# thelaycon/lazzaro

Hardware: AMD Instinct MI355X
Metric: search_memories QPS + recall@10 on 10M x d=768 index; consolidate turns/sec (higher is better)
Workload: dtype bf16 encoder; int8 scan -> bf16 re-score -> fp32 re-rank; 1 GPU; global_batch=1024, seq_len=32, parallelism=tenant-dp1

## Files before the change

csrc/kernels/search256.hip:

```cpp
#include "lzk_g256.h"
#include "lzk_i8score.h"

#include <cstdlib>
#include <cfloat>
#include <map>
#include <mutex>

LZK_DEBUG_STATE(search256)

namespace {

using namespace g256;

constexpr int kStampTiles = 32;
__device__ unsigned long long* g_stamps = nullptr;

template <bool HAS_BIAS, bool HAS_LABEL>
__global__ __launch_bounds__(NT, 1) void flat_cand_kernel(
    const u16* __restrict__ X, long ldx, int nrows, const u16* __restrict__ Qm, long ldq, int nq, int D,
    const float* __restrict__ bias, const int* __restrict__ row_label, const int* __restrict__ q_label,
    float alpha, const float* __restrict__ thr, int n_qt, int cap, int* __restrict__ cnt,
    float* __restrict__ cs, int* __restrict__ ci) {
  extern __shared__ __attribute__((aligned(16))) u16 smem[];
  const int logical = xcd_remap(blockIdx.x, gridDim.x);
// ... 554 lines not shown
    int mr = 0x7fffffff;
#pragma unroll
    for (int i = 0; i < 8; ++i) {
      const int rb = r0 + wr * 128 + i * 16 + 4 * (lane >> 4);
#pragma unroll
      for (int e = 0; e < 4; ++e) {
        const float v = acc[i][j][e];
        if (rb + e < nrows && v > m) { m = v; mr = rb + e; }
      }
    }
#pragma unroll
    for (int off = 16; off <= 32; off <<= 1) {
      const float om = __shfl_xor(m, off);
      const int orr = __shfl_xor(mr, off);
      if (om > m || (om == m && orr < mr)) { m = om; mr = orr; }
    }
    const int q = q0 + wc * 64 + j * 16 + (lane & 15);
    if ((lane >> 4) == 0 && q < nq && mr < nrows) atomicMax(best + q, top1_pack(m, mr));
  }
}

__global__ __launch_bounds__(NT, 1) void flat_top1_grouped_kernel(const u16* __restrict__ C, long ldc,
                                                                  const u16* __restrict__ Xq, long ldx,
                                                                  const int* __restrict__ qidx,
                                                                  const int4* __restrict__ blocks, int D,
                                                                  unsigned long long* __restrict__ best) {
  extern __shared__ __attribute__((aligned(16))) u16 smem[];
  const int4 bd = blocks[xcd_remap(blockIdx.x, gridDim.x)];
  const int c0 = bd.x, nc = bd.y, p0 = bd.z, np = bd.w;
  Stager st;
  st.setup(C + (long)c0 * ldc, ldc, 0, nc, Xq, ldx, 0, 1);
  {
    const int wave = __builtin_amdgcn_readfirstlane(threadIdx.x >> 6);
    const int lane = threadIdx.x & 63;
#pragma unroll
    for (int i = 0; i < 2; ++i) {
      const int row = 8 * (wave * 2 + i) + (lane >> 3);
      const int kc = (lane & 7) ^ ((row >> 1) & 7);
      LZK_DCHECK(qidx[p0 + min(row, np - 1)] >= 0);
      st.src[2][i] = Xq + (long)qidx[p0 + min(row, np - 1)] * ldx + kc * 8;
      st.src[3][i] = Xq + (long)qidx[p0 + min(128 + row, np - 1)] * ldx + kc * 8;
    }
  }
  f32x4 acc[8][4];
  mainloop(smem, st, D / BK, acc);

  const int lane = threadIdx.x & 63;
  const int wave = __builtin_amdgcn_readfirstlane(threadIdx.x >> 6);
  const int wr = wave >> 2, wc = wave & 3;
#pragma unroll
  for (int j = 0; j < 4; ++j) {
    float m = LZK_NEG_INF;
    int mr = 0x7fffffff;
#pragma unroll
    for (int i = 0; i < 8; ++i) {
      const int rb = wr * 128 + i * 16 + 4 * (lane >> 4);
#pragma unroll
      for (int e = 0; e < 4; ++e) {
        const float v = acc[i][j][e];
        if (rb + e < nc && v > m) { m = v; mr = rb + e; }
      }
    }
#pragma unroll
    for (int off = 16; off <= 32; off <<= 1) {
      const float om = __shfl_xor(m, off);
      const int orr = __shfl_xor(mr, off);
      if (om > m || (om == m && orr < mr)) { m = om; mr = orr; }
    }
    const int q = wc * 64 + j * 16 + (lane & 15);
    if ((lane >> 4) == 0 && q < np && mr < nc) atomicMax(best + p0 + q, top1_pack(m, c0 + mr));
  }
}

__global__ __launch_bounds__(256) void top1_decode_kernel(const unsigned long long* __restrict__ best, int nq,
                                                          float* __restrict__ score, int* __restrict__ row) {
  const int q = blockIdx.x * 256 + threadIdx.x;
  if (q >= nq) return;
  const unsigned long long b = best[q];
  if (b == 0ull) { score[q] = LZK_NEG_INF; row[q] = -1; return; }
  const unsigned key = (unsigned)(b >> 32);
  const unsigned u = (key & 0x80000000u) ? (key & 0x7fffffffu) : ~key;
  score[q] = __uint_as_float(u);
  row[q] = (int)(0xFFFFFFFFu - (unsigned)(b & 0xFFFFFFFFull));
}

template <bool F32>
__device__ __forceinline__ void load4(const void* p, long off, float (&v)[4]) {
  if constexpr (F32) {
    const float4 u = *reinterpret_cast<const float4*>(reinterpret_cast<const float*>(p) + off);
    v[0] = u.x; v[1] = u.y; v[2] = u.z; v[3] = u.w;
  } else {
    const uint2 u = *reinterpret_cast<const uint2*>(reinterpret_cast<const u16*>(p) + off);
    v[0] = __uint_as_float(u.x << 16); v[1] = __uint_as_float(u.x & 0xffff0000u);
    v[2] = __uint_as_float(u.y << 16); v[3] = __uint_as_float(u.y & 0xffff0000u);
  }
}

template <bool F32>
__global__ __launch_bounds__(256) void cand_rescore_kernel(const void* __restrict__ X, long ldx,
                                                           const void* __restrict__ Qm, long ldq, int D,
                                                           const float* __restrict__ bias, float alpha,
                                                           const int* __restrict__ cnt, int cap,
                                                           float* __restrict__ cs, const int* __restrict__ ci,
                                                           const float* __restrict__ cut, float floor,
                                                           const float* __restrict__ tau, int k_need,
                                                           int need_val, int* __restrict__ need,
                                                           int* __restrict__ hitc, int* __restrict__ done) {
  __shared__ int s_hits;
  const int q = blockIdx.x;
  const int lane = threadIdx.x & 63, wave = threadIdx.x >> 6;
  const int split = gridDim.y;
  if (threadIdx.x == 0) s_hits = 0;
  __syncthreads();
  const float tq = tau ? tau[q] : LZK_NEG_INF;
  int hits = 0;
  const int n = min(cnt[q] & 0x3fffffff, cap);
  const int chunks = D >> 2;
  constexpr int MAXC = 8;
  float qv[MAXC][4];
#pragma unroll
  for (int t = 0; t < MAXC; ++t) {
    const int c = lane + 64 * t;
    if (c < chunks) load4<F32>(Qm, (long)q * ldq + 4 * c, qv[t]);
  }
  const float cq = cut ? cut[q] : LZK_NEG_INF;
  for (int base = blockIdx.y * 256 + wave * 64; base < n; base += 256 * split) {
    const long li = (long)q * cap + base + lane;
    bool keep = base + lane < n;
    if (keep && cut) {
      keep = cs[li] >= cq;
      if (!keep) cs[li] = LZK_NEG_INF;
    }
    unsigned long long live = __ballot(keep);
    while (live) {
    const int jj = __builtin_ctzll(live);
    live &= live - 1;
    const long idx = (long)q * cap + base + jj;
    const int r = ci[idx];
    LZK_DCHECK(r >= 0);
    float acc = 0.f;
#pragma unroll
    for (int t = 0; t < MAXC; ++t) {
      const int c = lane + 64 * t;
      if (c < chunks) {
        float xv[4];
        load4<F32>(X, (long)r * ldx + 4 * c, xv);
        acc = fmaf(qv[t][0], xv[0], acc);
        acc = fmaf(qv[t][1], xv[1], acc);
        acc = fmaf(qv[t][2], xv[2], acc);
        acc = fmaf(qv[t][3], xv[3], acc);
      }
    }
#pragma unroll
    for (int o = 32; o >= 1; o >>= 1) acc += __shfl_xor(acc, o, 64);
    const float sc = alpha * acc + (bias ? bias[r] : 0.f);
    if (lane == 0) cs[idx] = sc >= floor ? sc : LZK_NEG_INF;
    hits += (sc >= floor && sc >= tq) ? 1 : 0;
    }
  }
  if (need) {
    if (lane == 0 && hits) atomicAdd(&s_hits, hits);
    __syncthreads();
    if (threadIdx.x == 0) {
      int tot = s_hits;
      bool last = true;
      if (split > 1) {
// ... 515 lines not shown
    if (hipMalloc(&s.p, (size_t)cap * sizeof(int)) != hipSuccess) {
      s.cap = 0;
      return nullptr;
    }
    s.cap = cap;
  }
  if (hipMemsetAsync(s.p, 0, (size_t)2 * nq * sizeof(int), st) != hipSuccess) return nullptr;
  return s.p;
}

template <bool F32>
int launch_rescore(const void* X, long ldx, const void* Q, long ldq, int nq, int D, const float* bias, float alpha,
                   const int* cnt, int cap, float* cs, const int* ci, const float* cut, float floor, const float* tau,
                   int k_need, int need_val, int* need, hipStream_t st) {
  int split = rescore_split(nq);
  int* ctr = nullptr;
  if (split > 1 && need) {
    ctr = rescore_counters(nq, st);
    if (!ctr) split = 1;
  }
  if (split > 1)
    hipLaunchKernelGGL(cand_rescore4_kernel<F32>, dim3((unsigned)nq, (unsigned)split), dim3(256), 0, st, X, ldx, Q,
                       ldq, D, bias, alpha, cnt, cap, cs, ci, cut, floor, tau, k_need, need_val, need, ctr,
                       ctr ? ctr + nq : nullptr);
  else
    hipLaunchKernelGGL(cand_rescore_kernel<F32>, dim3((unsigned)nq, 1u), dim3(256), 0, st, X, ldx, Q, ldq, D, bias,
                       alpha, cnt, cap, cs, ci, cut, floor, tau, k_need, need_val, need, ctr, ctr ? ctr + nq : nullptr);
  return (int)hipGetLastError();
}
}

LZK_EXPORT int lzk_cand_rescore(const void* X16, long ldx, const void* Q16, long ldq, int nq, int D, const float* bias,
                                float alpha, const int* cnt, int cap, float* cs, const int* ci, const float* cut,
                                float floor, const float* tau, int k_need, int need_val, int* need, void* stream) {
  if (D % 4 != 0 || D > 2048 || nq <= 0) return (int)hipErrorInvalidValue;
  return launch_rescore<false>(X16, ldx, Q16, ldq, nq, D, bias, alpha, cnt, cap, cs, ci, cut, floor, tau, k_need,
                               need_val, need, (hipStream_t)stream);
}

LZK_EXPORT int lzk_cand_rescore32(const float* X32, long ldx, const float* Q32, long ldq, int nq, int D,
                                  const float* bias, float alpha, const int* cnt, int cap, float* cs, const int* ci,
                                  const float* cut, float floor, const float* tau, int k_need, int need_val,
                                  int* need, void* stream) {
  if (D % 4 != 0 || D > 2048 || nq <= 0 || ldx % 4 != 0 || ldq % 4 != 0) return (int)hipErrorInvalidValue;
  return launch_rescore<true>(X32, ldx, Q32, ldq, nq, D, bias, alpha, cnt, cap, cs, ci, cut, floor, tau, k_need,
                              need_val, need, (hipStream_t)stream);
}

__global__ __launch_bounds__(256) void thr_prep_kernel(const float* __restrict__ ts, long ldts, int col,
                                                       const float* __restrict__ margin,
                                                       const float* __restrict__ margin_rig, int nq,
                                                       float* __restrict__ thr, float* __restrict__ cert,
                                                       int* __restrict__ cnt) {
#pragma clang fp contract(off)
  const int q = blockIdx.x * 256 + threadIdx.x;
  if (q >= nq) return;
  float t = ts[(long)q * ldts + col];
  const float sl = 1.0f + fabsf(t);
  t = t - 2e-4f * sl;
  if (t != t) t = LZK_NEG_INF;
  else if (t == LZK_NEG_INF) t = -FLT_MAX;
  else if (t == __builtin_inff()) t = FLT_MAX;
  const float th = margin ? t - margin[q] : t;
  thr[q] = th;
  if (cert) {
    float c = margin_rig ? th + margin_rig[q] : th;
    const float cs = 1.0f + fabsf(c);
    c = c + 1e-6f * cs;
    if (c != c) c = LZK_NEG_INF;
    else if (c == __builtin_inff()) c = FLT_MAX;
    cert[q] = c;
  }
  if (cnt) cnt[q] = 0;
}

LZK_EXPORT int lzk_thr_prep(const float* ts, long ldts, int col, const float* margin, const float* margin_rig, int nq,
                            float* thr, float* cert, int* cnt, void* stream) {
  if (nq <= 0 || col < 0 || col >= ldts || !ts || !thr) return (int)hipErrorInvalidValue;
  hipLaunchKernelGGL(thr_prep_kernel, dim3((unsigned)((nq + 255) / 256)), dim3(256), 0, (hipStream_t)stream, ts, ldts,
                     col, margin, margin_rig, nq, thr, cert, cnt);
  return (int)hipGetLastError();
}

LZK_EXPORT int lzk_cand_cut(const void* X, long ldx, long nrows, const void* Q, long ldq, int D, int nq, int f32,
                            const float* bias, float alpha, const long* rows, int ldr, int k, const float* margin,
                            float floor, int has_floor, float* cut, void* stream) {
  if (D % 4 != 0 || D > 2048 || nq <= 0 || k <= 0 || k > ldr || !margin) return (int)hipErrorInvalidValue;
  if (f32 && (ldx % 4 != 0 || ldq % 4 != 0)) return (int)hipErrorInvalidValue;
  const dim3 grid((unsigned)((nq + 3) / 4)), block(256);
  if (nq < 64 && k <= 16) {
    if (f32)
      hipLaunchKernelGGL(cand_cut_block_kernel<true>, dim3((unsigned)nq), dim3(1024), 0, (hipStream_t)stream, X, ldx,
                         nrows, Q, ldq, D, nq, bias, alpha, rows, ldr, k, margin, floor, has_floor, cut);
    else
      hipLaunchKernelGGL(cand_cut_block_kernel<false>, dim3((unsigned)nq), dim3(1024), 0, (hipStream_t)stream, X,
                         ldx, nrows, Q, ldq, D, nq, bias, alpha, rows, ldr, k, margin, floor, has_floor, cut);
    return (int)hipGetLastError();
  }
  if (f32)
    hipLaunchKernelGGL(cand_cut_kernel<true>, grid, block, 0, (hipStream_t)stream, X, ldx, nrows, Q, ldq, D, nq,
                       bias, alpha, rows, ldr, k, margin, floor, has_floor, cut);
  else
    hipLaunchKernelGGL(cand_cut_kernel<false>, grid, block, 0, (hipStream_t)stream, X, ldx, nrows, Q, ldq, D, nq,
                       bias, alpha, rows, ldr, k, margin, floor, has_floor, cut);
  return (int)hipGetLastError();
}

LZK_EXPORT int lzk_flat_cand_i8(const void* X8, long ldx_bytes, int nrows, const void* Q8, long ldq_bytes, int nq,
                                int D_bytes, const float* bias, const float* rscale, const float* qscale, float alpha,
                                const float* thr, int cap, int* cnt, float* cs, int* ci, void* blk_buf, int blk_cap,
                                int* blk_cnt, void* stream) {
  if (D_bytes % 128 != 0 || D_bytes > 1024 || (ldx_bytes | ldq_bytes) % 16 != 0 || nq <= 0 || nrows <= 0 ||
      cap <= 0 || !rscale || !qscale || !(alpha > 0.f))
    return (int)hipErrorInvalidValue;
  if (!blk_buf || blk_cap <= 0 || !blk_cnt) return (int)hipErrorInvalidValue;
  const BlkCands blk{(int4*)blk_buf, blk_cap, blk_cnt, rscale, qscale};
  const int n_rt = (nrows + BM - 1) / BM, n_qt = (nq + BN - 1) / BN;
  const long nblk = (long)n_rt * n_qt;
  if (nblk > 0x7fffffffL) return (int)hipErrorInvalidValue;
  const int ncu = n_cu();
  const int grid = (int)(nblk < ncu ? nblk : ncu);
  hipStream_t st = (hipStream_t)stream;
  const u16* x = (const u16*)X8;
  const u16* q = (const u16*)Q8;
  const int* rs = nullptr;
  const int* qs = nullptr;
#define LZK_GIO(B, O)                                                                                               \
  do {                                                                                                              \
    (void)hipFuncSetAttribute((const void*)flat_cand_persistent_kernel<B, false, false, O, MmaI8>,                  \
                              hipFuncAttributeMaxDynamicSharedMemorySize, CAND_P_LDS);                              \
    hipLaunchKernelGGL((flat_cand_persistent_kernel<B, false, false, O, MmaI8>), dim3(grid), dim3(NT), CAND_P_LDS, \
                       st, x, ldx_bytes / 2, nrows, q, ldq_bytes / 2, nq, D_bytes / 2, bias, rs, qs, alpha, thr,    \
                       n_qt, (int)nblk, cap, cnt, cs, ci, (const float*)nullptr, (int*)nullptr, (float*)nullptr,    \
                       (int*)nullptr, blk);                                                                         \
  } while (0)
#define LZK_GIS(B)                              \
  do {                                          \
    switch (g_i8_opt) {                         \
      case 28: LZK_GIO(B, 28); break;           \
      case 8: LZK_GIO(B, 8); break;             \
      case 24: LZK_GIO(B, 24); break;           \
      case 88: LZK_GIO(B, 88); break;           \
      default: LZK_GIO(B, kI8Opt); break;       \
    }                                           \
  } while (0)
  if (bias) LZK_GIS(true);
  else LZK_GIS(false);
#undef LZK_GIS
#undef LZK_GIO
  return (int)hipGetLastError();
}

LZK_EXPORT int lzk_flat_cand_dual_i8(const void* X8, long ldx_bytes, int nrows, const void* Q8, long ldq_bytes,
                                     int nq, int D_bytes, const float* bias, const float* rscale,
                                     const float* qscale, const int* row_label, const int* q_label, float alpha,
                                     const float* thr, const float* thr2, int cap, int* cnt, float* cs, int* ci,
                                     int* cnt2, float* cs2, int* ci2, void* blk_buf, int blk_cap, int* blk_cnt,
                                     void* stream) {
  if (D_bytes % 128 != 0 || D_bytes > 1024 || (ldx_bytes | ldq_bytes) % 16 != 0 || nq <= 0 || nrows <= 0 ||
      cap <= 0 || !rscale || !qscale || !row_label || !q_label || !(alpha > 0.f))
    return (int)hipErrorInvalidValue;
  if (!blk_buf || blk_cap <= 0 || !blk_cnt) return (int)hipErrorInvalidValue;
  const BlkCands blk{(int4*)blk_buf, blk_cap, blk_cnt, rscale, qscale};
  const int n_rt = (nrows + BM - 1) / BM, n_qt = (nq + BN - 1) / BN;
  const long nblk = (long)n_rt * n_qt;
  if (nblk > 0x7fffffffL) return (int)hipErrorInvalidValue;
// ... 29 lines not shown
```

lazzaro_amd/ops/search.py:

```python
from __future__ import annotations

import math
import os

import numpy as np
import torch

from . import _lib

TARGET_WGS = 512


def _ref_topk(X, Q, k, bias=None, row_label=None, q_label=None, alpha=1.0, idx_offset=0,
              chunk=1 << 16):
    nq = Q.shape[0]
    n = X.shape[0]
    dev = X.device
    best_s = torch.full((nq, 0), float("-inf"), device=dev)
    best_i = torch.zeros((nq, 0), dtype=torch.long, device=dev)
    Qf = Q.float()
    for c0 in range(0, n, chunk):
        c1 = min(n, c0 + chunk)
        s = alpha * (Qf @ X[c0:c1].float().T)
        if bias is not None:
# ... 391 lines not shown
    thr = _sample_threshold(X16, Q16, k, kslot, bias, None, None, alpha, S)
    if margin is not None:
        thr = (thr - margin).contiguous()
    cap = max(2048, 32 * kslot * S)
    cnt, cs, ci = _cand_lists(dev, nq, cap, 0)
    grid = L.lzk_cand_grid_f8(N, nq)
    bbuf, bcap, bcnt = _blk_records(dev, grid, nq, kslot, 4 * S, 1)
    st = _lib.stream_ptr(dev)
    _lib.check(L.lzk_flat_cand_f8(X8.data_ptr(), X8.stride(0), N, Q8.data_ptr(), Q8.stride(0), nq, Dp, _lib.ptr(bias),
                                  float(alpha / scale2), thr.data_ptr(), cap, cnt.data_ptr(), cs.data_ptr(),
                                  ci.data_ptr(), bbuf.data_ptr(), bcap, bcnt.data_ptr(), st), "lzk_flat_cand_f8")
    _lib.check(L.lzk_cand_gather(bbuf.data_ptr(), bcap, bcnt.data_ptr(), grid, cap, nq, cnt.data_ptr(), cs.data_ptr(),
                                 ci.data_ptr(), None, None, None, st), "lzk_cand_gather")
    _lib.check(L.lzk_cand_rescore(X16.data_ptr(), X16.stride(0), Q16.data_ptr(), Q16.stride(0), nq, Dp,
                                  _lib.ptr(bias), float(alpha), cnt.data_ptr(), cap, cs.data_ptr(), ci.data_ptr(), None,
                                  float("-inf"), None, 0, 0, None, st), "lzk_cand_rescore")
    return _select_with_fallback(X16, Q16, k, kslot, bias, None, None, alpha, 0, cnt, cs, ci, cap)


def quantize_i8_rows(x: torch.Tensor, out: torch.Tensor = None, scale_out: torch.Tensor = None):
    xf = x.float()
    amax = xf.abs().amax(1)
    s = torch.where(amax > 0, amax / 127.0, torch.zeros_like(amax))
    den = torch.where(amax > 0, s, torch.ones_like(amax))
    q = torch.round(xf / den[:, None]).clamp_(-127, 127).to(torch.int8)
    if out is not None:
        out[:, : q.shape[1]] = q
        q = out
    if scale_out is not None:
        scale_out.copy_(s)
        s = scale_out
    return q, s


def i8_query(q16: torch.Tensor, d: int, sumsq: torch.Tensor, n_sumsq: int, smax: torch.Tensor, alpha: float,
             z: float, xn: float = 1.0):
    nq, Dp = q16.shape
    dev = q16.device
    q8 = torch.empty((nq, Dp), dtype=torch.int8, device=dev)
    qs = torch.empty(nq, dtype=torch.float32, device=dev)
    margin = torch.empty(nq, dtype=torch.float32, device=dev)
    margin_rig = torch.empty(nq, dtype=torch.float32, device=dev)
    q16 = q16.contiguous()
    _lib.check(_lib.lib().lzk_i8_query(q16.data_ptr(), q16.stride(0), nq, Dp, int(d), sumsq.data_ptr(),
                                       1.0 / max(int(n_sumsq), 1), smax.data_ptr(), abs(float(alpha)), float(z),
                                       float(xn), q8.data_ptr(), q8.stride(0), qs.data_ptr(), margin.data_ptr(),
                                       margin_rig.data_ptr(), _lib.stream_ptr(dev)), "lzk_i8_query")
    return q8, qs, margin, margin_rig


I8_SAMPLE = os.environ.get("LZK_I8_SAMPLE", "1") != "0"
_lib.register("lzk_sample_topk_i8", _lib.I, [_lib.P, _lib.L, _lib.I, _lib.I, _lib.P, _lib.L, _lib.I, _lib.P, _lib.P,
                                             _lib.P, _lib.F, _lib.I, _lib.I, _lib.I, _lib.P, _lib.P, _lib.P])


def sample_topk_i8(X8: torch.Tensor, rscale: torch.Tensor, Q8: torch.Tensor, qscale: torch.Tensor, kslot: int,
                   S: int, *, bias=None, alpha: float = 1.0, n_chunks: int = None):
    L = _lib.lib()
    nq, Dp = Q8.shape
    N = X8.shape[0]
    dev = X8.device
    assert X8.dtype == torch.int8 and Q8.dtype == torch.int8 and Dp % 128 == 0 and Dp <= 1024 and X8.shape[1] == Dp
    assert X8.stride(1) == 1 and Q8.stride(1) == 1 and N > 0 and nq > 0 and S >= 1
    assert rscale.dtype == torch.float32 and rscale.stride(0) == 1 and rscale.shape[0] >= N
    assert bias is None or (bias.dtype == torch.float32 and bias.stride(0) == 1 and bias.shape[0] >= N)
    qs = qscale.contiguous()
    assert qs.dtype == torch.float32 and qs.shape[0] == nq
    ns = -(-N // S)
    if n_chunks:
        rpc = -(-(-(-ns // n_chunks)) // 128) * 128
        nch = -(-ns // rpc)
    else:
        nch = L.lzk_flat_topk_chunks(ns, nq, TARGET_WGS)
    part = nq * nch * kslot
    ws = _ws.get(dev, part * 8)
    ps = ws[: part * 4].view(torch.float32)
    pi = ws[part * 4: part * 8].view(torch.int32)
    _lib.check(L.lzk_sample_topk_i8(X8.data_ptr(), X8.stride(0), N, int(S), Q8.data_ptr(), Q8.stride(0), nq,
                                    rscale.data_ptr(), qs.data_ptr(), _lib.ptr(bias), float(alpha), Dp, kslot, nch,
                                    ps.data_ptr(), pi.data_ptr(), _lib.stream_ptr(dev)), "lzk_sample_topk_i8")
    return _merge_partials(ps, pi, nch, nq, kslot, kslot, 0)


def flat_topk_i8(X8: torch.Tensor, rscale: torch.Tensor, Q8: torch.Tensor, qscale: torch.Tensor,
                 X16: torch.Tensor, Q16: torch.Tensor, k: int, *, bias=None, alpha: float = 1.0, margin=None,
                 margin_rig=None):
    L = _lib.lib()
    nq, Dp = Q16.shape
    N = X16.shape[0]
    kslot = L.lzk_flat_topk_kslot(int(k))
    assert kslot > 0 and X8.dtype == torch.int8 and Q8.dtype == torch.int8 and Dp % 128 == 0 and Dp <= 1024
    assert X8.shape[1] == Dp and X8.stride(1) == 1 and Q8.stride(1) == 1 and X8.shape[0] >= N
    assert rscale.dtype == torch.float32 and qscale.dtype == torch.float32 and rscale.shape[0] >= N
    assert alpha > 0
    dev = X16.device
    if margin_rig is None:
        margin_rig = margin
    narrow = nq < NARROW_MAX_Q and SCAN8_NARROW and Dp % 64 == 0
    S = max(1, min(CAND_STRIDE_NARROW if narrow else CAND_STRIDE, N // max(16 * kslot, 1)))
    J = SPEC_J_NARROW if narrow else SPEC_J
    spec = 0 < J < k and S >= SPEC_MIN_STRIDE
    if I8_SAMPLE:
        ts, _ = sample_topk_i8(X8[:N], rscale, Q8, qscale, kslot, S, bias=bias, alpha=alpha)
    else:
        bs = bias[:N:S].contiguous() if bias is not None else None
        ts, _ = _flat_topk_lane(X16[::S], Q16, kslot, kslot, bs, None, None, alpha, 0, None)
    cap = max(NARROW_CAP if narrow else 2048, 16 * kslot * S)
    cnt, cs, ci = _cand_lists(dev, nq, cap, 0, zero=False)
    thr = torch.empty(nq, dtype=torch.float32, device=dev)
    cert = torch.empty(nq, dtype=torch.float32, device=dev)
    mg = margin.float().contiguous() if margin is not None else None
    mr = margin_rig.float().contiguous() if margin_rig is not None else None
    _lib.check(L.lzk_thr_prep(ts.data_ptr(), ts.stride(0), (J if spec else k) - 1, _lib.ptr(mg), _lib.ptr(mr), nq,
                              thr.data_ptr(), cert.data_ptr(), cnt.data_ptr(), _lib.stream_ptr(dev)), "lzk_thr_prep")
    qs = qscale.contiguous()
    need = torch.empty(nq, dtype=torch.int32, device=dev)
    chk = (cert, k, cap + 1, need)
    if narrow:
        _scan8_narrow(X8[:N], rscale[:N], Q8, qs, bias, alpha, thr, kslot, 2 * S, cap, (cnt, cs, ci))
    else:
        grid = L.lzk_cand_grid_f8(N, nq)
        bbuf, bcap, bcnt = _blk_records(dev, grid, nq, kslot, 2 * S, 1)
        st = _lib.stream_ptr(dev)
        _lib.check(L.lzk_flat_cand_i8(X8.data_ptr(), X8.stride(0), N, Q8.data_ptr(), Q8.stride(0), nq, Dp,
                                      _lib.ptr(bias), rscale.data_ptr(), qs.data_ptr(), float(alpha), thr.data_ptr(),
                                      cap, cnt.data_ptr(), cs.data_ptr(), ci.data_ptr(), bbuf.data_ptr(), bcap,
                                      bcnt.data_ptr(), st), "lzk_flat_cand_i8")
        _lib.check(L.lzk_cand_gather(bbuf.data_ptr(), bcap, bcnt.data_ptr(), grid, cap, nq, cnt.data_ptr(),
                                     cs.data_ptr(), ci.data_ptr(), None, None, None, st), "lzk_cand_gather")
    _rescore_above_cut(X16, Q16, k, kslot, bias, alpha, margin_rig, cnt, cs, ci, cap, chk=chk)
    return _select_with_fallback(X16, Q16, k, kslot, bias, None, None, alpha, 0, cnt, cs, ci, cap, need=need)


_lib.register("lzk_cand_select_wide", _lib.I, [_lib.P, _lib.P, _lib.P, _lib.I, _lib.I, _lib.I, _lib.L, _lib.P, _lib.P,
                                               _lib.P, _lib.P, _lib.P, _lib.P])
_lib.register("lzk_flat_topk_wide_chunks", _lib.I, [_lib.I, _lib.I])
_lib.register("lzk_flat_topk_wide", _lib.I, [_lib.P, _lib.L, _lib.I, _lib.P, _lib.L, _lib.I, _lib.P, _lib.F, _lib.I,
                                             _lib.I, _lib.P, _lib.P, _lib.I, _lib.L, _lib.P, _lib.P, _lib.P])
_lib.register("lzk_flat_topk_wide_masked", _lib.I, [_lib.P, _lib.L, _lib.I, _lib.P, _lib.L, _lib.I, _lib.P, _lib.F,
                                                    _lib.I, _lib.I, _lib.P, _lib.P, _lib.I, _lib.L, _lib.P, _lib.P,
                                                    _lib.P, _lib.P])

WIDE_K_MAX = 64
WIDE_P_FALLBACK = 1e-4
WIDE_J = None
WIDE_CAP_MIN = 2048
WIDE_LIST_FACTOR = 16
_ws_wide = _Workspace()


def wide_spec_j(k: int, S: int, p_max: float = WIDE_P_FALLBACK) -> int:
    k, S = int(k), max(int(S), 1)
    p = 1.0 / S
    for j in range(1, 17):
        tail = sum(math.comb(k, i) * p ** i * (1.0 - p) ** (k - i) for i in range(j, k + 1))
        if tail <= p_max:
            return j
    return 16


def _wide_chunks(N: int, nq: int, n_chunks=None) -> int:
    hint = int(n_chunks) if n_chunks else min(-(-N // 8192), max(8, min(256, 65536 // max(nq, 1))))
    return _lib.lib().lzk_flat_topk_wide_chunks(int(N), max(hint, 1))


def _flat_topk_wide(X16, Q16, k, bias, alpha, idx_offset=0, n_chunks=None, q_active=None, out=None):
    L = _lib.lib()
    nq, D = Q16.shape
    N = X16.shape[0]
    dev = X16.device
    assert X16.dtype == torch.bfloat16 and Q16.dtype == torch.bfloat16 and 1 <= k <= WIDE_K_MAX
    assert X16.shape[1] == D and D % 8 == 0 and D <= 2048 and X16.stride(1) == 1 and Q16.stride(1) == 1
    assert bias is None or (bias.dtype == torch.float32 and bias.is_contiguous() and bias.shape[0] >= N)
    if out is None:
        assert q_active is None
        out = (torch.empty((nq, k), dtype=torch.float32, device=dev), torch.empty((nq, k), dtype=torch.long, device=dev))
    os_, oi = out
    nch = _wide_chunks(N, nq, n_chunks)
    part = nq * nch * WIDE_K_MAX
    ws = _ws_wide.get(dev, part * 8)
    ps = ws[: part * 4].view(torch.float32)
    pi = ws[part * 4: part * 8].view(torch.int32)
    args = (X16.data_ptr(), X16.stride(0), N, Q16.data_ptr(), Q16.stride(0), nq, _lib.ptr(bias), float(alpha), D,
            nch, ps.data_ptr(), pi.data_ptr(), int(k), int(idx_offset), os_.data_ptr(), oi.data_ptr())
    if q_active is None:
        _lib.check(L.lzk_flat_topk_wide(*args, _lib.stream_ptr(dev)), "lzk_flat_topk_wide")
    else:
        assert q_active.dtype == torch.int32 and q_active.shape[0] == nq
        _lib.check(L.lzk_flat_topk_wide_masked(*args, q_active.data_ptr(), _lib.stream_ptr(dev)),
                   "lzk_flat_topk_wide_masked")
    return os_, oi


def flat_topk_wide(X16: torch.Tensor, Q16: torch.Tensor, k: int, *, bias=None, alpha: float = 1.0,
                   idx_offset: int = 0, n_chunks: int = None):
    if Q16.dim() == 1:
        Q16 = Q16[None, :]
    if not X16.is_cuda:
        return _ref_topk(X16, Q16, k, bias, None, None, alpha, idx_offset)
    nq = Q16.shape[0]
    if X16.shape[0] == 0 or nq == 0:
        return (torch.full((nq, k), float("-inf"), device=X16.device),
                torch.full((nq, k), -1, dtype=torch.long, device=X16.device))
    return _flat_topk_wide(X16, Q16, k, bias, alpha, idx_offset, n_chunks)


def cand_select_wide(cnt, cs, ci, cap: int, kout: int, *, idx_offset: int = 0, need=None, q_active=None, out=None):
    nq = cs.shape[0] if cs.dim() == 2 else cs.numel() // cap
    dev = cs.device
    if out is None:
        out = (torch.empty((nq, kout), dtype=torch.float32, device=dev),
               torch.empty((nq, kout), dtype=torch.long, device=dev))
    ovf = torch.empty((nq,), dtype=torch.int32, device=dev)
    _lib.check(_lib.lib().lzk_cand_select_wide(_lib.ptr(cnt), cs.data_ptr(), ci.data_ptr(), int(cap), nq, int(kout),
                                               int(idx_offset), out[0].data_ptr(), out[1].data_ptr(), ovf.data_ptr(),
                                               _lib.ptr(need), _lib.ptr(q_active), _lib.stream_ptr(dev)),
               "lzk_cand_select_wide")
    return out[0], out[1], ovf


def flat_topk_i8_wide(X8: torch.Tensor, rscale: torch.Tensor, Q8: torch.Tensor, qscale: torch.Tensor,
                      X16: torch.Tensor, Q16: torch.Tensor, k: int, *, bias=None, alpha: float = 1.0, margin=None,
                      margin_rig=None):
    k = int(k)
    assert 16 < k <= WIDE_K_MAX, "flat_topk_i8_wide serves 17 <= k <= 64 (flat_topk_i8 below)"
    if not X16.is_cuda:
        return _ref_topk(X16, Q16, k, bias, None, None, alpha, 0)
    L = _lib.lib()
    nq, Dp = Q16.shape
    N = X16.shape[0]
    kslot = 16
    assert X8.dtype == torch.int8 and Q8.dtype == torch.int8 and Dp % 128 == 0 and Dp <= 1024
    assert X8.shape[1] == Dp and X8.stride(1) == 1 and Q8.stride(1) == 1 and X8.shape[0] >= N
    assert rscale.dtype == torch.float32 and qscale.dtype == torch.float32 and rscale.shape[0] >= N
    assert alpha > 0 and not isinstance(X16, LeanRows)
    dev = X16.device
    st = _lib.stream_ptr(dev)
    if margin_rig is None:
        margin_rig = margin
    narrow = nq < NARROW_MAX_Q and SCAN8_NARROW and Dp % 64 == 0
    S = max(1, min(CAND_STRIDE_NARROW if narrow else CAND_STRIDE, N // max(16 * kslot, 1)))
    j = int(WIDE_J) if WIDE_J else wide_spec_j(k, S)
    ts, _ = sample_topk_i8(X8[:N], rscale, Q8, qscale, kslot, S, bias=bias, alpha=alpha)
    cap = max(NARROW_CAP if narrow else WIDE_CAP_MIN, WIDE_LIST_FACTOR * j * S, WIDE_K_MAX)
    cnt, cs, ci = _cand_lists(dev, nq, cap, 0, zero=False)
    thr = torch.empty(nq, dtype=torch.float32, device=dev)
    cert = torch.empty(nq, dtype=torch.float32, device=dev)
    mg = margin.float().contiguous() if margin is not None else None
    mr = margin_rig.float().contiguous() if margin_rig is not None else None
    _lib.check(L.lzk_thr_prep(ts.data_ptr(), ts.stride(0), j - 1, _lib.ptr(mg), _lib.ptr(mr), nq, thr.data_ptr(),
                              cert.data_ptr(), cnt.data_ptr(), st), "lzk_thr_prep")
    qs = qscale.contiguous()
    need = torch.empty(nq, dtype=torch.int32, device=dev)
    if narrow:
        _scan8_narrow(X8[:N], rscale[:N], Q8, qs, bias, alpha, thr, j, 2 * S, cap, (cnt, cs, ci))
    else:
        grid = L.lzk_cand_grid_f8(N, nq)
        bbuf, bcap, bcnt = _blk_records(dev, grid, nq, j, 2 * S, 1)
        _lib.check(L.lzk_flat_cand_i8(X8.data_ptr(), X8.stride(0), N, Q8.data_ptr(), Q8.stride(0), nq, Dp,
                                      _lib.ptr(bias), rscale.data_ptr(), qs.data_ptr(), float(alpha), thr.data_ptr(),
                                      cap, cnt.data_ptr(), cs.data_ptr(), ci.data_ptr(), bbuf.data_ptr(), bcap,
                                      bcnt.data_ptr(), st), "lzk_flat_cand_i8")
        _lib.check(L.lzk_cand_gather(bbuf.data_ptr(), bcap, bcnt.data_ptr(), grid, cap, nq, cnt.data_ptr(),
                                     cs.data_ptr(), ci.data_ptr(), None, None, None, st), "lzk_cand_gather")
    _rescore_above_cut_wide(X16, Q16, k, bias, alpha, mr, cnt, cs, ci, cap, (cert, k, cap + 1, need))
    return _select_with_fallback_wide(X16, Q16, k, bias, alpha, cnt, cs, ci, cap, need=need)


def _rescore_above_cut_wide(X16, Q16, k, bias, alpha, margin, cnt, cs, ci, cap, chk):
    L = _lib.lib()
    nq, Dp = Q16.shape
    dev = Q16.device
    st = _lib.stream_ptr(dev)
    tau, k_need, need_val, need = chk
    cut = None
    if margin is not None:
        _, i8, _ = cand_select_wide(cnt, cs, ci, cap, k)
        cut = torch.empty(nq, dtype=torch.float32, device=dev)
        _lib.check(L.lzk_cand_cut(X16.data_ptr(), X16.stride(0), int(X16.shape[0]), Q16.data_ptr(), Q16.stride(0),
                                  Dp, nq, 0, _lib.ptr(bias), float(alpha), i8.data_ptr(), k, k, margin.data_ptr(),
                                  0.0, 0, cut.data_ptr(), st), "lzk_cand_cut")
    _lib.check(L.lzk_cand_rescore(X16.data_ptr(), X16.stride(0), Q16.data_ptr(), Q16.stride(0), nq, Dp,
                                  _lib.ptr(bias), float(alpha), cnt.data_ptr(), cap, cs.data_ptr(), ci.data_ptr(),
                                  _lib.ptr(cut), float("-inf"), tau.data_ptr(), int(k_need), int(need_val),
                                  need.data_ptr(), st), "lzk_cand_rescore")


def _select_with_fallback_wide(X16, Q16, k, bias, alpha, cnt, cs, ci, cap, need=None, ovf_sink=None):
    os_, oi, ovf = cand_select_wide(cnt, cs, ci, cap, k, need=need)
    if ovf_sink is not None:
        ovf_sink.append((ovf, cnt))
    return _flat_topk_wide(X16, Q16, k, bias, alpha, 0, None, q_active=ovf, out=(os_, oi))


def _cert_tau(thr: torch.Tensor, margin_rig: torch.Tensor, floor: float = None,
              floor_tol: float = 0.0) -> torch.Tensor:
    t = thr + margin_rig if margin_rig is not None else thr
    fl_ok = (t <= float(floor) + float(floor_tol)) if floor is not None else None
    t = t + 1e-6 * (1.0 + t.abs())
    if fl_ok is not None:
        t = torch.where(fl_ok, torch.full_like(t, float("-inf")), t)
    return torch.nan_to_num(t, nan=float("-inf"), neginf=float("-inf")).contiguous()


SPEC_J = 5
SPEC_J_NARROW = 3
NARROW_CAP = 16384
SPEC_MIN_STRIDE = 32
SPEC_STATS = [] if os.environ.get("LZK_SPEC_STATS") == "1" else None


def _rescore_above_cut(X16, Q16, k, kslot, bias, alpha, margin, cnt, cs, ci, cap, floor=None, chk=None):
    tau_p, k_need, need_val, need_p = (None, 0, 0, None) if chk is None else (
        chk[0].data_ptr(), int(chk[1]), int(chk[2]), chk[3].data_ptr())
    L = _lib.lib()
    nq, Dp = Q16.shape
    dev = Q16.device
    st = _lib.stream_ptr(dev)
    cut = None
    if margin is not None:
        s8 = torch.empty((nq, kslot), dtype=torch.float32, device=dev)
        i8 = torch.empty((nq, kslot), dtype=torch.long, device=dev)
        ovf = torch.empty((nq,), dtype=torch.int32, device=dev)
        _lib.check(L.lzk_cand_select(cnt.data_ptr(), cs.data_ptr(), ci.data_ptr(), cap, nq, kslot, kslot, 0,
                                     s8.data_ptr(), i8.data_ptr(), ovf.data_ptr(), None, st), "lzk_cand_select")
        cut = torch.empty(nq, dtype=torch.float32, device=dev)
# ... 341 lines not shown
```

Baseline: 85750 queries/s.

## Replace sampled top-k threshold with per-group max then select

Adds a sampled int8 GEMM kernel that writes only a per-128-row-group maximum score per query, instead of full per-chunk top-k partials. A small select kernel then picks the top kslot group maxima to form the threshold. The goal is to cut the cost of the sampling stage (partial top-k maintenance and the merge). The resulting threshold is a lower bound that differs from the true k-th sampled score, which may let more candidates through the later stages. It is enabled by default when there are enough groups, and the epilogue scales and bias are staged into LDS asynchronously.

```diff
diff --git a/csrc/kernels/search256.hip b/csrc/kernels/search256.hip
--- a/csrc/kernels/search256.hip
+++ b/csrc/kernels/search256.hip
@@ -660,6 +660,152 @@
   const unsigned u = (key & 0x80000000u) ? (key & 0x7fffffffu) : ~key;
   score[q] = __uint_as_float(u);
   row[q] = (int)(0xFFFFFFFFu - (unsigned)(b & 0xFFFFFFFFull));
+}
+
+constexpr int GMAX_ARRAYS = 3;
+constexpr int GMAX_LDS = LDS_BYTES + 2 * GMAX_ARRAYS * 256 * 4;
+
+template <bool HAS_BIAS, bool STAGED>
+__global__ __launch_bounds__(NT, 1) void sample_gmax_i8_kernel(
+    const u16* __restrict__ X, long lds_row, int ns, long S, const u16* __restrict__ Qm, long ldq, int nq, int D,
+    const float* __restrict__ rscale, const float* __restrict__ bias, const float* __restrict__ qscale, float alpha,
+    int n_qt, int n_tiles, float* __restrict__ gmax, long ldg) {
+  typedef int i32x4 __attribute__((ext_vector_type(4)));
+  extern __shared__ __attribute__((aligned(16))) u16 smem[];
+  float* epi = reinterpret_cast<float*>(smem + EPI_OFF);
+  const int lane = threadIdx.x & 63;
+  const int wave = __builtin_amdgcn_readfirstlane(threadIdx.x >> 6);
+  const int wr = wave >> 2, wc = wave & 3;
+  const int KS = D / BK;
+
+  TileWalk walk;
+  walk.init(n_tiles);
+  int tile = walk.next;
+  if (!walk.valid(tile)) return;
+
+  auto stage_epi = [&](int tl, int par) {
+    if constexpr (STAGED) {
+      const int r0 = (tl / n_qt) * BM, q0 = (tl % n_qt) * BN;
+#pragma unroll
+      for (int g = wave; g < 4 * GMAX_ARRAYS; g += 8) {
+        const int a = g >> 2, c = g & 3;
+        if (a == 1 && !HAS_BIAS) continue;
+        const long r = (long)min(r0 + c * 64 + lane, ns - 1) * S;
+        const float* src;
+        if (a == 0) src = rscale + r;
+        else if (a == 1) src = bias + r;
+        else src = qscale + min(q0 + c * 64 + lane, nq - 1);
+        __builtin_amdgcn_global_load_lds((gbl_void_t*)src,
+                                         (lds_void_t*)(epi + par * (GMAX_ARRAYS * 256) + a * 256 + c * 64), 4, 0, 0);
+      }
+    }
+  };
+
+  Stager st;
+  st.setup(X, lds_row, (tile / n_qt) * BM, ns, Qm, ldq, (tile % n_qt) * BN, nq);
+  auto ex0 = [&]() { stage_epi(tile, 0); };
+  prologue<decltype(ex0), 8>(smem, st, KS, ex0);
+  int par = 0;
+  f32x4 acc[8][4];
+  while (true) {
+    const int cur = tile, cpar = par;
+    tile += walk.step;
+    const bool more = walk.valid(tile);
+    body2<MmaI8>(smem, st, KS, acc, true);
+    if (more) {
+      st.setup(X, lds_row, (tile / n_qt) * BM, ns, Qm, ldq, (tile % n_qt) * BN, nq);
+      auto exn = [&]() { stage_epi(tile, cpar ^ 1); };
+      prologue<decltype(exn), 8>(smem, st, KS, exn);
+    }
+    const int r0 = (cur / n_qt) * BM, q0 = (cur % n_qt) * BN;
+    const float* e_rs = epi + cpar * (GMAX_ARRAYS * 256);
+    const float* e_bias = e_rs + 256;
+    const float* e_qs = e_rs + 512;
+    const bool full = r0 + BM <= ns;
+    float al[4], m[4];
+#pragma unroll
+    for (int j = 0; j < 4; ++j) {
+      const int qlo = wc * 64 + j * 16 + (lane & 15);
+      al[j] = alpha * (STAGED ? e_qs[qlo] : qscale[min(q0 + qlo, nq - 1)]);
+      m[j] = LZK_NEG_INF;
+    }
+#pragma unroll
+    for (int i = 0; i < 8; ++i) {
+      const int rl = wr * 128 + i * 16 + 4 * (lane >> 4);
+      f32x4 rs, bv = {0.f, 0.f, 0.f, 0.f};
+      if constexpr (STAGED) {
+        rs = *reinterpret_cast<const f32x4*>(e_rs + rl);
+        if (HAS_BIAS) bv = *reinterpret_cast<const f32x4*>(e_bias + rl);
+      } else {
+#pragma unroll
+        for (int e = 0; e < 4; ++e) {
+          const long r = (long)min(r0 + rl + e, ns - 1) * S;
+          rs[e] = rscale[r];
+          if (HAS_BIAS) bv[e] = bias[r];
+        }
+      }
+#pragma unroll
+      for (int j = 0; j < 4; ++j) {
+        const i32x4 v = __builtin_bit_cast(i32x4, acc[i][j]);
+#pragma unroll
+        for (int e = 0; e < 4; ++e) {
+          float sc = i8_score(al[j], i8_prod(v[e], rs[e]), bv[e]);
+          if (!(full || r0 + rl + e < ns)) sc = LZK_NEG_INF;
+          m[j] = fmaxf(m[j], sc);
+        }
+      }
+    }
+    float* out = gmax + (long)(2 * (r0 / BM) + wr) * ldg;
+#pragma unroll
+    for (int j = 0; j < 4; ++j) {
+      float mm = fmaxf(m[j], __shfl_xor(m[j], 16, 64));
+      mm = fmaxf(mm, __shfl_xor(mm, 32, 64));
+      const int q = q0 + wc * 64 + j * 16 + (lane & 15);
+      if ((lane >> 4) == 0 && q < nq) out[q] = mm;
+    }
+    if (!more) break;
+    par = cpar ^ 1;
+  }
+}
+
+template <int K>
+__global__ __launch_bounds__(256) void gmax_select_kernel(const float* __restrict__ gmax, long ldg, int G, int nq,
+                                                          float* __restrict__ ts) {
+  const int lane = threadIdx.x & 63;
+  const int q = blockIdx.x * 4 + (threadIdx.x >> 6);
+  if (q >= nq) return;
+  TopK<K> top;
+  top.init();
+  constexpr int U = 8;
+  for (int g0 = 0; g0 < G; g0 += 64 * U) {
+    float v[U];
+#pragma unroll
+    for (int u = 0; u < U; ++u) {
+      const int g = g0 + u * 64 + lane;
+      v[u] = g < G ? gmax[(long)g * ldg + q] : LZK_NEG_INF;
+    }
+#pragma unroll
+    for (int u = 0; u < U; ++u)
+      if (g0 + u * 64 + lane < G) top.push(v[u], g0 + u * 64 + lane);
+  }
+  for (int j = 0; j < K; ++j) {
+    const float hs = top.s[0];
+    const int hi = top.i[0];
+    float bs = hs;
+    int bi = hi;
+#pragma unroll
+    for (int o = 32; o >= 1; o >>= 1) {
+      const float s2 = __shfl_xor(bs, o, 64);
+      const int i2 = __shfl_xor(bi, o, 64);
+      if (better(s2, i2, bs, bi)) { bs = s2; bi = i2; }
+    }
+    if (lane == 0) ts[(long)q * K + j] = (bi == 0x7fffffff) ? LZK_NEG_INF : bs;
+    if (hi == bi && hs == bs && bi != 0x7fffffff) {
+#pragma unroll
+      for (int t = 0; t < K - 1; ++t) { top.s[t] = top.s[t + 1]; top.i[t] = top.i[t + 1]; }
+      top.s[K - 1] = LZK_NEG_INF; top.i[K - 1] = 0x7fffffff;
+    }
+  }
 }
 
 template <bool F32>
@@ -1341,6 +1487,59 @@
   return (int)hipGetLastError();
 }
 
+int g_gmax_opt = 0;
+LZK_EXPORT void lzk_set_gmax_opt(int v) { g_gmax_opt = v; }
+
+LZK_EXPORT int lzk_sample_gmax_i8(const void* X8, long ldx_bytes, int nrows, int S, const void* Q8, long ldq_bytes,
+                                  int nq, int D_bytes, const float* rscale, const float* qscale, const float* bias,
+                                  float alpha, int kslot, float* gmax, long ldg, int n_groups, float* ts,
+                                  void* stream) {
+  if (D_bytes % 128 != 0 || D_bytes <= 0 || D_bytes > 1024 || (ldx_bytes | ldq_bytes) % 16 != 0 ||
+      ldx_bytes < D_bytes || ldq_bytes < D_bytes || ((uintptr_t)X8 | (uintptr_t)Q8) % 16 != 0 || nq <= 0 ||
+      nrows <= 0 || S <= 0 || !rscale || !qscale || !gmax || !ts || ldg < nq)
+    return (int)hipErrorInvalidValue;
+  if (kslot != 1 && kslot != 2 && kslot != 4 && kslot != 8 && kslot != 10 && kslot != 16)
+    return (int)hipErrorInvalidValue;
+  const int ns = (int)(((long)nrows + S - 1) / S);
+  const int n_rt = (ns + BM - 1) / BM, n_qt = (nq + BN - 1) / BN;
+  const long nblk = (long)n_rt * n_qt;
+  if (nblk > 0x7fffffffL || n_groups != 2 * n_rt) return (int)hipErrorInvalidValue;
+  const int ncu = n_cu();
+  const int grid = (int)(nblk < ncu ? nblk : ncu);
+  hipStream_t st = (hipStream_t)stream;
+#define LZK_GMX(B, T)                                                                                                \
+  do {                                                                                                               \
+    (void)hipFuncSetAttribute((const void*)sample_gmax_i8_kernel<B, T>, hipFuncAttributeMaxDynamicSharedMemorySize,  \
+                              GMAX_LDS);                                                                             \
+    hipLaunchKernelGGL((sample_gmax_i8_kernel<B, T>), dim3(grid), dim3(NT), GMAX_LDS, st, (const u16*)X8,            \
+                       (long)S * (ldx_bytes / 2), ns, (long)S, (const u16*)Q8, ldq_bytes / 2, nq, D_bytes / 2,       \
+                       rscale, bias, qscale, alpha, n_qt, (int)nblk, gmax, ldg);                                     \
+  } while (0)
+  if (g_gmax_opt == 1) {
+    if (bias) LZK_GMX(true, false);
+    else LZK_GMX(false, false);
+  } else {
+    if (bias) LZK_GMX(true, true);
+    else LZK_GMX(false, true);
+  }
+#undef LZK_GMX
+  int rc = (int)hipGetLastError();
+  if (rc) return rc;
+  const dim3 sgrid((unsigned)((nq + 3) / 4)), sblock(256);
+#define LZK_GSEL(KK) hipLaunchKernelGGL(gmax_select_kernel<KK>, sgrid, sblock, 0, st, gmax, ldg, n_groups, nq, ts)
+  switch (kslot) {
+    case 1: LZK_GSEL(1); break;
+    case 2: LZK_GSEL(2); break;
+    case 4: LZK_GSEL(4); break;
+    case 8: LZK_GSEL(8); break;
+    case 10: LZK_GSEL(10); break;
+    case 16: LZK_GSEL(16); break;
+    default: return (int)hipErrorInvalidValue;
+  }
+#undef LZK_GSEL
+  return (int)hipGetLastError();
+}
+
 LZK_EXPORT int lzk_cand_cut(const void* X, long ldx, long nrows, const void* Q, long ldq, int D, int nq, int f32,
                             const float* bias, float alpha, const long* rows, int ldr, int k, const float* margin,
                             float floor, int has_floor, float* cut, void* stream) {
diff --git a/lazzaro_amd/ops/search.py b/lazzaro_amd/ops/search.py
--- a/lazzaro_amd/ops/search.py
+++ b/lazzaro_amd/ops/search.py
@@ -497,6 +497,52 @@
     return _merge_partials(ps, pi, nch, nq, kslot, kslot, 0)
 
 
+I8_GMAX = os.environ.get("LZK_I8_GMAX", "1") != "0"
+SAMPLE_MODE = "auto"
+GMAX_MIN_GROUPS = 8
+_lib.register("lzk_sample_gmax_i8", _lib.I, [_lib.P, _lib.L, _lib.I, _lib.I, _lib.P, _lib.L, _lib.I, _lib.I, _lib.P,
+                                             _lib.P, _lib.P, _lib.F, _lib.I, _lib.P, _lib.L, _lib.I, _lib.P, _lib.P])
+
+
+def gmax_groups(N: int, S: int) -> int:
+    return 2 * -(-(-(-int(N) // int(S))) // 256)
+
+
+def _use_gmax(N: int, S: int, kslot: int, narrow: bool) -> bool:
+    if narrow or not I8_SAMPLE or SAMPLE_MODE == "topk":
+        return False
+    if SAMPLE_MODE == "gmax":
+        return True
+    return I8_GMAX and gmax_groups(N, S) >= GMAX_MIN_GROUPS * kslot
+
+
+def sample_gmax_i8(X8: torch.Tensor, rscale: torch.Tensor, Q8: torch.Tensor, qscale: torch.Tensor, kslot: int,
+                   S: int, *, bias=None, alpha: float = 1.0):
+    L = _lib.lib()
+    nq, Dp = Q8.shape
+    N = X8.shape[0]
+    dev = X8.device
+    assert X8.dtype == torch.int8 and Q8.dtype == torch.int8 and Dp % 128 == 0 and Dp <= 1024 and X8.shape[1] == Dp
+    assert X8.stride(1) == 1 and Q8.stride(1) == 1 and N > 0 and nq > 0 and S >= 1
+    assert rscale.dtype == torch.float32 and rscale.stride(0) == 1 and rscale.shape[0] >= N
+    assert bias is None or (bias.dtype == torch.float32 and bias.stride(0) == 1 and bias.shape[0] >= N)
+    qs = qscale.contiguous()
+    assert qs.dtype == torch.float32 and qs.shape[0] == nq
+    G = gmax_groups(N, S)
+    gm = _ws.get(dev, G * nq * 4)
+    ts = torch.empty((nq, kslot), dtype=torch.float32, device=dev)
+    _lib.check(L.lzk_sample_gmax_i8(X8.data_ptr(), X8.stride(0), N, int(S), Q8.data_ptr(), Q8.stride(0), nq, Dp,
+                                    rscale.data_ptr(), qs.data_ptr(), _lib.ptr(bias), float(alpha), kslot,
+                                    gm.data_ptr(), nq, G, ts.data_ptr(), _lib.stream_ptr(dev)), "lzk_sample_gmax_i8")
+    return ts
+
+
+def _i8_sample(X8, rscale, Q8, qscale, kslot, S, narrow, bias, alpha):
+    if _use_gmax(X8.shape[0], S, kslot, narrow):
+        return sample_gmax_i8(X8, rscale, Q8, qscale, kslot, S, bias=bias, alpha=alpha)
+    return sample_topk_i8(X8, rscale, Q8, qscale, kslot, S, bias=bias, alpha=alpha)[0]
+
+
 def flat_topk_i8(X8: torch.Tensor, rscale: torch.Tensor, Q8: torch.Tensor, qscale: torch.Tensor,
                  X16: torch.Tensor, Q16: torch.Tensor, k: int, *, bias=None, alpha: float = 1.0, margin=None,
                  margin_rig=None):
@@ -516,7 +562,7 @@
     J = SPEC_J_NARROW if narrow else SPEC_J
     spec = 0 < J < k and S >= SPEC_MIN_STRIDE
     if I8_SAMPLE:
-        ts, _ = sample_topk_i8(X8[:N], rscale, Q8, qscale, kslot, S, bias=bias, alpha=alpha)
+        ts = _i8_sample(X8[:N], rscale, Q8, qscale, kslot, S, narrow, bias, alpha)
     else:
         bs = bias[:N:S].contiguous() if bias is not None else None
         ts, _ = _flat_topk_lane(X16[::S], Q16, kslot, kslot, bs, None, None, alpha, 0, None)
@@ -656,7 +702,7 @@
     narrow = nq < NARROW_MAX_Q and SCAN8_NARROW and Dp % 64 == 0
     S = max(1, min(CAND_STRIDE_NARROW if narrow else CAND_STRIDE, N // max(16 * kslot, 1)))
     j = int(WIDE_J) if WIDE_J else wide_spec_j(k, S)
-    ts, _ = sample_topk_i8(X8[:N], rscale, Q8, qscale, kslot, S, bias=bias, alpha=alpha)
+    ts = _i8_sample(X8[:N], rscale, Q8, qscale, kslot, S, narrow, bias, alpha)
     cap = max(NARROW_CAP if narrow else WIDE_CAP_MIN, WIDE_LIST_FACTOR * j * S, WIDE_K_MAX)
     cnt, cs, ci = _cand_lists(dev, nq, cap, 0, zero=False)
     thr = torch.empty(nq, dtype=torch.float32, device=dev)
```

Measured after the change: 86730 queries/s, median of 6. 1.1% higher.
